# aayush9400/3D-Condtional-Stable-Diffusion

Measured on AMD Instinct MI355X. Metric: latent volumes/sec at 32^3x8ch T=1000 DDPM, higher is better.
Workload: dtype f32 (f16 hi+lo x3 MFMA, f32 accumulate)

## Files before the change

3d-condtional-stable-diffusion_amd/_lib.py:

```python
from __future__ import annotations

import ctypes as C
import os

_HERE = os.path.dirname(os.path.abspath(__file__))
LIB_PATH = os.environ.get("DM3D_LIB") or os.path.join(_HERE, "csrc", "libdm3d_hip.so")

ACT_NONE, ACT_RELU, ACT_SILU = 0, 1, 2
ABI_VERSION = 111
PREC_F32, PREC_H3 = 0, 1
WL_TAP, WL_PAIR = 0, 1
FMT_F32, FMT_H2 = 0, 1
COUT_PAD, CIN_PAD = 64, 16

_f32p = C.c_void_p
_i32p = C.c_void_p


class ConvDesc(C.Structure):
    _fields_ = [
        ("x1", _f32p), ("x2", _f32p), ("c1", C.c_int32), ("c2", C.c_int32), ("batch", C.c_int32),
        ("in_d", C.c_int32), ("in_h", C.c_int32), ("in_w", C.c_int32), ("upsample", C.c_int32),
        ("ksize", C.c_int32), ("stride", C.c_int32), ("wpk", _f32p), ("bias", _f32p),
        ("pro_scale", _f32p), ("pro_shift", _f32p), ("vec", _f32p), ("vec_idx", _i32p), ("vec_ld", C.c_int32),
# ... 152 lines not shown
    "dm3d_split_h2": (C.c_int, [_f32p, C.c_int64, C.c_int32, C.c_int64, C.c_int32, C.c_void_p, C.c_int64, C.c_void_p]),
    "dm3d_layernorm3_h2": (C.c_int, [_f32p, C.c_int64, C.c_int32, C.c_float] + [_f32p] * 9 + [C.c_void_p]),
    "dm3d_softmax_rows_h2": (C.c_int, [_f32p, C.c_int64, C.c_int32, C.c_int64, C.c_void_p]),
    "dm3d_layernorm3": (C.c_int, [_f32p, C.c_int64, C.c_int32, C.c_float] + [_f32p] * 9 + [C.c_void_p]),
    "dm3d_groupnorm_stats": (C.c_int, [_f32p, C.c_int32, C.c_int64, C.c_int32, C.c_void_p, C.c_int32, C.c_int32, C.c_void_p]),
    "dm3d_groupnorm_finalize": (C.c_int, [C.c_void_p, C.c_int32, C.c_int64, C.c_int32, C.c_int32, C.c_float, _f32p, _f32p, _f32p,
                                           _f32p, C.c_void_p]),
    "dm3d_groupnorm_finalize2": (C.c_int, [C.c_void_p, C.c_int32, C.c_void_p, C.c_int32, C.c_int32, C.c_int64, C.c_int32, C.c_float, _f32p, _f32p,
                                          _f32p, _f32p, C.c_void_p]),
    "dm3d_groupnorm_partials": (C.c_int, [_f32p, C.c_int32, C.c_int64, C.c_int32, C.c_void_p, C.c_void_p]),
    "dm3d_groupnorm_partials_bytes": (C.c_int64, [C.c_int32, C.c_int64, C.c_int32]),
    "dm3d_affine_act_batched": (C.c_int, [_f32p, _f32p, C.c_int32, C.c_int64, C.c_int32, _f32p, _f32p, C.c_int32, C.c_void_p]),
    "dm3d_softmax_rows": (C.c_int, [_f32p, C.c_int64, C.c_int32, C.c_int64, C.c_void_p]),
    "dm3d_affine_act": (C.c_int, [_f32p, _f32p, C.c_int64, C.c_int32, _f32p, _f32p, C.c_int32, C.c_void_p]),
    "dm3d_ddpm_update": (C.c_int, [C.POINTER(DdpmDesc), C.c_void_p]),
    "dm3d_ddim_update": (C.c_int, [C.POINTER(DdimDesc), C.c_void_p]),
    "dm3d_dpm_update": (C.c_int, [C.POINTER(DpmDesc), C.c_void_p]),
    "dm3d_edit_update": (C.c_int, [C.POINTER(EditDesc), C.c_void_p]),
    "dm3d_guide_update": (C.c_int, [C.POINTER(GuideDesc), C.c_void_p]),
    "dm3d_range_check": (C.c_int, [_f32p, C.c_int64, C.c_float, C.c_void_p, C.c_void_p]),
    "dm3d_add_i32": (C.c_int, [_i32p, C.c_int32, C.c_int32, C.c_void_p]),
    "dm3d_randn": (C.c_int, [_f32p, C.c_int64, C.c_uint64, C.c_uint32, C.c_void_p]),
    "dm3d_gather_rows": (C.c_int, [_f32p, C.c_int32, _i32p, _f32p, C.c_int32, C.c_int32, C.c_void_p]),
    "dm3d_vq_assign": (C.c_int, [_f32p, C.c_int64, C.c_int32, _f32p, C.c_int32, _f32p, _i32p, C.c_void_p]),
    "dm3d_batchnorm_finalize": (C.c_int, [C.c_void_p, C.c_int32, C.c_int64, C.c_int32, C.c_float] + [_f32p] * 8 + [C.c_float, C.c_int32, C.c_void_p]),
    "dm3d_affine_act_cat": (C.c_int, [_f32p, C.c_int32, _f32p, C.c_int32, C.c_int64, _f32p, _f32p, C.c_int32, _f32p, C.c_void_p]),
    "dm3d_bn_act_bwd": (C.c_int, [_f32p, _f32p, C.c_int32, _f32p, C.c_int32, C.c_int64, _f32p, _f32p, _f32p, _f32p, C.c_int32, C.c_void_p,
                                   _f32p, _f32p, _f32p, _f32p, C.c_void_p]),
    "dm3d_wgrad": (C.c_int, [C.POINTER(WgradDesc), C.c_void_p]),
    "dm3d_colsum": (C.c_int, [_f32p, C.c_int64, C.c_int64, C.c_int32, _f32p, C.c_int64, C.c_void_p]),
# ... 77 lines not shown
```

3d-condtional-stable-diffusion_amd/csrc/dm3d_conv.hip:

```cpp
#include <cstdlib>
#include "dm3d_conv_args.h"
#include <math.h>

namespace {

template <int TD, int TH, int TW, int S, int KS, int WM, int WN>
__global__ __launch_bounds__(256, 2) void conv3d_igemm_f32(const ConvArgs p) {
    constexpr int CK = 16, LDV = CK + 4, NT = 64;
    constexpr int TM = TD * TH * TW;
    constexpr int HD = (TD - 1) * S + KS, HH = (TH - 1) * S + KS, HW = (TW - 1) * S + KS;
    constexpr int HVOX = HD * HH * HW;
    constexpr int TAPS = KS * KS * KS;
    constexpr int MR = TM / WM / 32, NR = NT / WN / 32;
    constexpr int NTHR = WM * WN * 64;
    constexpr int NSLOT = (HVOX * 4 + NTHR - 1) / NTHR;
    static_assert(NTHR == 256, "kernel assumes 4 waves");
    static_assert(TM % (WM * 32) == 0 && NT % (WN * 32) == 0, "tile split");

    extern __shared__ __attribute__((aligned(16))) float smem[];
    float* lds_in = smem;
    float* lds_w = smem + HVOX * LDV;

    const int tid = threadIdx.x;
    const int lane = tid & 63, wave = tid >> 6;
// ... 169 lines not shown
    int dev_ = 0;
    DM3D_HIP(hipGetDevice(&dev_));
    DM3D_REQUIRE(dev_ >= 0 && dev_ < 64, "conv: device ordinal %d", dev_);
    if (!attr_set[dev_]) {
        DM3D_HIP(hipFuncSetAttribute(reinterpret_cast<const void*>(&conv3d_igemm_f32<TD, TH, TW, S, KS, WM, WN>),
                                     hipFuncAttributeMaxDynamicSharedMemorySize, (int)lds));
        attr_set[dev_] = true;
    }
    dim3 grid((unsigned)(a.batch * a.bd * a.bh * a.bw), (unsigned)(a.coutpad / 64), a.parity ? 8u : 1u);
    hipLaunchKernelGGL((conv3d_igemm_f32<TD, TH, TW, S, KS, WM, WN>), grid, dim3(256), lds, st, a);
    return dm3d_launch_check("conv3d_igemm_f32");
}

}

extern "C" int dm3d_conv3d_ndhwc(const dm3d_conv_desc* d, void* stream) {
    DM3D_REQUIRE(d != nullptr, "conv: null descriptor");
    DM3D_REQUIRE(d->x1 && d->wpk && d->out, "conv: x1/wpk/out must be non-null");
    DM3D_REQUIRE(d->ksize == 1 || d->ksize == 3 || (d->ksize == 4 && d->stride == 2), "conv: ksize %d not in {1,3} (4 needs stride 2)", d->ksize);
    DM3D_REQUIRE(d->stride == 1 || d->stride == 2, "conv: stride %d not in {1,2}", d->stride);
    DM3D_REQUIRE(!d->transpose || (d->ksize == 4 && d->stride == 2 && !d->upsample), "conv: transpose needs ksize 4, stride 2, no upsample");
    DM3D_REQUIRE(!(d->upsample && d->stride != 1), "conv: upsample requires stride 1");
    DM3D_REQUIRE(!(d->ksize == 1 && (d->stride != 1 || d->upsample)), "conv: ksize 1 supports stride 1 without upsample only");
    DM3D_REQUIRE(d->batch > 0 && d->in_d > 0 && d->in_h > 0 && d->in_w > 0 && d->cout > 0, "conv: non-positive extent");
    DM3D_REQUIRE(d->c1 > 0 && d->c1 % 4 == 0 && d->c2 >= 0 && d->c2 % 4 == 0, "conv: c1=%d c2=%d must be multiples of 4", d->c1, d->c2);
    DM3D_REQUIRE((d->c2 == 0) == (d->x2 == nullptr), "conv: x2 and c2 must be given together");
    DM3D_REQUIRE(d->c2 == 0 || d->c1 % 16 == 0, "conv: with a second input c1=%d must be a multiple of 16", d->c1);
    DM3D_REQUIRE((d->pro_scale == nullptr) == (d->pro_shift == nullptr), "conv: pro_scale and pro_shift go together");
    DM3D_REQUIRE(!d->vec || d->vec_ld >= d->cout, "conv: vec_ld %d < cout %d", d->vec_ld, d->cout);
    const void* ptrs[] = {d->x1, d->x2, d->wpk, d->pro_scale, d->pro_shift, d->out, d->res};
    for (const void* q : ptrs) DM3D_REQUIRE(dm3d_aligned16(q), "conv: pointer %p is not 16-byte aligned", q);
// ... 68 lines not shown
    a.out_scale = d->precision == DM3D_PREC_H3 ? ldexpf(1.0f, -d->w_exp) : 1.0f;
    hipStream_t st = static_cast<hipStream_t>(stream);
    const int which = par_mode ? DM3D_CONV_UP
                               : (d->ksize == 1 ? DM3D_CONV_K1 : (d->ksize == 4 ? DM3D_CONV_K4S2 : (d->stride == 2 ? DM3D_CONV_K3S2 : DM3D_CONV_K3S1)));
    if (par_mode) a.w_parity_stride = d->precision == DM3D_PREC_H3
        ? dm3d_packed_weight_h3_bytes(8, cin, d->cout) / 2 : dm3d_packed_weight_elems(8, cin, d->cout);
    if (d->gn_stats) {
        DM3D_REQUIRE(d->out_fmt == DM3D_FMT_F32 && d->cout % 4 == 0 && dm3d_aligned16(d->gn_stats),
                     "conv: gn_stats needs a float32 output, cout %% 4 == 0 and a 16-byte aligned buffer");
        a.gn_stats = d->gn_stats;
    }
    auto stats_behind = [&](int rc) {
        if (rc != DM3D_OK || !a.gn_stats) return rc;
        return dm3d_groupnorm_partials(a.out, a.batch, (int64_t)a.fd * a.fh * a.fw, a.cout, a.gn_stats, stream);
    };
    if (d->precision != DM3D_PREC_H3) return stats_behind(dm3d_conv_launch_f32(a, which, st));
    const int layout = dm3d_conv_weight_layout(d->ksize, d->stride, d->upsample, d->transpose, d->cout);
    DM3D_REQUIRE(d->w_layout == layout, "conv: w_layout %d but this geometry reads layout %d (dm3d_conv_weight_layout)", d->w_layout, layout);
    if (layout != DM3D_WL_PAIR) return stats_behind(dm3d_conv_launch_h3(a, which, st));
    if (dm3d_conv_h3w_serves(a, which)) return dm3d_conv_launch_h3w(a, which, st);
    return dm3d_conv_launch_h3v3(a, which, st);
}

extern "C" int64_t dm3d_packed_weight_skip_h3p_bytes(int32_t cin, int32_t cout) {
    return (cin > 0 && cout > 0) ? dm3d_h3v2_skip_image_bytes(cin, cout) : 0;
}

extern "C" int dm3d_pack_weights_skip_h3p(const float* keras_kernel, int32_t cin, int32_t cout, int32_t w_exp, void* packed, void* stream) {
    DM3D_REQUIRE(keras_kernel && packed && cin > 0 && cout > 0, "pack_weights_skip_h3p: bad arguments");
    DM3D_REQUIRE(w_exp >= -100 && w_exp <= 100 && dm3d_aligned16(packed), "pack_weights_skip_h3p: w_exp out of range or packed unaligned");
    return dm3d_pack_skip_h3v2(keras_kernel, cin, cout, w_exp, packed, static_cast<hipStream_t>(stream));
}

extern "C" int dm3d_pack_weights_skip_h3f(const float* keras_kernel, int32_t cin, int32_t cout, int32_t w_exp, void* packed, void* stream) {
    DM3D_REQUIRE(keras_kernel && packed && cin > 0 && cout > 0, "pack_weights_skip_h3f: bad arguments");
    DM3D_REQUIRE(w_exp >= -100 && w_exp <= 100 && dm3d_aligned16(packed), "pack_weights_skip_h3f: w_exp out of range or packed unaligned");
// ... 100 lines not shown
```

3d-condtional-stable-diffusion_amd/csrc/dm3d_conv_args.h:

```cpp
#pragma once
#include "dm3d_common.h"

struct ConvArgs {
    const float* x1; const float* x2; int c1, c2;
    int ind, inh, inw;
    int lgd, lgh, lgw;
    int od, oh, ow;
    int padz, pady, padx;
    int os;
    int ooz, ooy, oox;
    int fd, fh, fw;
    int parity;
    long w_parity_stride;
    const void* wpk; int cinpad, coutpad;
    const float* bias; const float* pscale; const float* pshift; long pro_bstride;
    const float* vec; const int* vec_idx; int vec_ld;
    int relu; const float* res; float* out; int cout;
    const float* prelu; int relu_out;
    int bd, bh, bw;
    int nchunks;
    int batch;
    float out_scale;
    int ksplit;
    int* split_counters;
    int split_counter_words;
    long split_tile_floats;
    void* scratch; long scratch_bytes;
    const float* post_scale; const float* post_shift;
    int out_h2;
    int x_h2;
    const float* sx1; const float* sx2; int sc1, sc2; const void* swpk; int s_npairs;
    const void* swpk_f;
    const void* wpk_wino;
    int* range_flag; float range_limit;
    float* gn_stats;
    int epi_vec4;
};

enum { DM3D_CONV_K3S1 = 0, DM3D_CONV_K3S2 = 1, DM3D_CONV_K1 = 2, DM3D_CONV_UP = 3, DM3D_CONV_K4S2 = 4 };

int dm3d_conv_launch_f32(ConvArgs& a, int which, hipStream_t st);
int dm3d_conv_launch_h3(ConvArgs& a, int which, hipStream_t st);
int dm3d_conv_launch_h3v3(ConvArgs& a, int which, hipStream_t st);
struct H3v2Launch { ConvArgs k; bool stats_after; };
int dm3d_h3v2_pre_launch(ConvArgs& a, int td, H3v2Launch& L, hipStream_t st, int force_ksplit = 0);
int dm3d_h3v2_post_launch(const ConvArgs& a, const H3v2Launch& L, hipStream_t st);
int dm3d_conv_h3v2_ksplit(const ConvArgs& a);
long dm3d_conv_split_tiles(const ConvArgs& a, int td);
int dm3d_conv_h3v3_td(const ConvArgs& a);
int64_t dm3d_h3v2_skip_image_bytes(int cin, int cout);
int dm3d_pack_skip_h3v2(const float* keras_kernel, int cin, int cout, int w_exp, void* packed, hipStream_t st);
// ... 8 lines not shown
```

3d-condtional-stable-diffusion_amd/csrc/dm3d_conv_h3v2_parts.h:

```cpp
#pragma once
#include "dm3d_conv_args.h"
#include "dm3d_h3.h"
#include <type_traits>

namespace h3v2 {

constexpr int REC = DM3D_REC;
typedef float f32x4v __attribute__((ext_vector_type(4)));

__host__ __device__ constexpr int pi_pos(int c) {
    return c < 4 ? (c < 2 ? c : c + 2) : (c >= 12 ? (c < 14 ? c - 4 : c - 2) : (((c - 4) >> 1) * 4 + 2 + ((c - 4) & 1)));
}
__device__ __forceinline__ int dx_of_row(int i) { return (0x1320 >> ((i >> 2) * 4)) & 3; }

#define DM3D_MFMA3_TILES(acc, nb, al, ah, bl, bh)                                                        \
    _Pragma("unroll") for (int pi_ = 0; pi_ < 4; ++pi_)                                                  \
        _Pragma("unroll") for (int k_ = 0; k_ < 2; ++k_) {                                               \
            f32x4v& c_ = acc[pi_][(nb) * 2 + k_];                                                        \
            c_ = __builtin_amdgcn_mfma_f32_16x16x32_f16(al[pi_], bh[k_], c_, 0, 0, 0);                   \
            c_ = __builtin_amdgcn_mfma_f32_16x16x32_f16(ah[pi_], bl[k_], c_, 0, 0, 0);                   \
            c_ = __builtin_amdgcn_mfma_f32_16x16x32_f16(ah[pi_], bh[k_], c_, 0, 0, 0);                   \
        }

struct Brick {
// ... 401 lines not shown
        for (int ni = 0; ni < NCT; ++ni) {
            *reinterpret_cast<f32x4*>(dst + ni * 32) = f32x4{gn[ni * 8], gn[ni * 8 + 1], gn[ni * 8 + 2], gn[ni * 8 + 3]};
            *reinterpret_cast<f32x4*>(dst + ni * 32 + 4) = f32x4{gn[ni * 8 + 4], gn[ni * 8 + 5], gn[ni * 8 + 6], gn[ni * 8 + 7]};
        }
        for (int k = 1; k < slices; ++k) {
            float* dz = dst + (size_t)k * bh * bw * p.cout * 2;
#pragma unroll
            for (int ni = 0; ni < NCT; ++ni) {
                *reinterpret_cast<f32x4*>(dz + ni * 32) = f32x4{0.f, 0.f, 0.f, 0.f};
                *reinterpret_cast<f32x4*>(dz + ni * 32 + 4) = f32x4{0.f, 0.f, 0.f, 0.f};
            }
        }
    }
}

struct EpiVecs { f32x4 add, ps, pt; };
__device__ __forceinline__ EpiVecs epilogue_cq_vecs(const ConvArgs& p, const Brick& br, const int vrow) {
    int tid = threadIdx.x;
    asm volatile("" : "+v"(tid));
    const int n = br.ntile * 64 + (tid & 15) * 4;
    const f32x4 zero = {0.f, 0.f, 0.f, 0.f}, one = {1.f, 1.f, 1.f, 1.f};
    EpiVecs ev;
    ev.add = zero; ev.ps = one; ev.pt = zero;
    if (br.ntile * 64 + 64 <= p.cout && p.epi_vec4) {
        if (p.bias) ev.add = *reinterpret_cast<const f32x4*>(p.bias + n);
        if (p.vec) {
            const f32x4 vv = *reinterpret_cast<const f32x4*>(p.vec + (size_t)vrow * p.vec_ld + n);
#pragma unroll
            for (int c = 0; c < 4; ++c) ev.add[c] += vv[c];
        }
// ... 122 lines not shown
```

3d-condtional-stable-diffusion_amd/csrc/dm3d_conv_h3v3.hip:

```cpp
#include <cstdlib>
#include "dm3d_conv_h3v2_parts.h"

using namespace h3v2;

#ifdef DM3D_CLOCK_STAMPS
__device__ unsigned long long* g_dbg_stamps_c = nullptr;
extern "C" int dm3d_debug_set_stamps_conv(void* p) { return (int)hipMemcpyToSymbol(HIP_SYMBOL(g_dbg_stamps_c), &p, sizeof(p)); }
#define STAMP(i) do { const unsigned wg_ = blockIdx.x + gridDim.x * blockIdx.y; \
    if (g_dbg_stamps_c && threadIdx.x == 0 && blockIdx.z == 0 && wg_ < 4096) { \
    g_dbg_stamps_c[wg_ * 32 + (i)] = __builtin_amdgcn_s_memtime(); \
    if ((i) == 0) g_dbg_stamps_c[wg_ * 32 + 24] = __builtin_amdgcn_s_memrealtime(); \
    if ((i) == 20) g_dbg_stamps_c[wg_ * 32 + 26] = __builtin_amdgcn_s_memrealtime(); \
    if ((i) == 29) g_dbg_stamps_c[wg_ * 32 + 25] = __builtin_amdgcn_s_memrealtime(); \
    if ((i) == 1) g_dbg_stamps_c[wg_ * 32 + 30] = __builtin_amdgcn_s_memrealtime(); \
    if ((i) == 28) g_dbg_stamps_c[wg_ * 32 + 31] = __builtin_amdgcn_s_memrealtime(); } } while (0)
#else
#define STAMP(i) do { } while (0)
#endif

namespace {

template <int KS, int MODE, int TD, int NCT = 4>
__global__ __launch_bounds__(TD * 64, 2) void conv3d_igemm_h3v3(const ConvArgs p) {
    constexpr int TH = 8, TW = 8, CK = 16, NT = 64, NTHR = TD * 64;
// ... 322 lines not shown
    const Brick br = {b, oz0, oy0, ox0, ooz, ooy, oox, ntile, khalf};
    if constexpr (KS == 3 && NCT == 4) {
        skip_phase<TD>(p, smem_v3, acc, br);
    }
    STAMP(19);
    if (p.ksplit > 1) {
        const long tile = ((long)blockIdx.z * gridDim.x + brick_all) * ntiles + ntile;
        const SplitTile stile = split_tile(p, tile, khalf);
        split_store(stile, acc, 0);
        STAMP(20);
        if (!split_is_last(p, tile, reinterpret_cast<unsigned*>(smem_v3))) return;
        STAMP(21);
        split_gather(stile, p, khalf, acc, 0);
        STAMP(22);
    }
    if (p.gn_stats) {
        float gn[NCT * 8];
#pragma unroll
        for (int i = 0; i < NCT * 8; ++i) gn[i] = 0.0f;
        epilogue<TD, NCT>(p, acc, br, -1, 4, -1, gn);
        gn_flush<TD, NCT>(p, gn, br, threadIdx.x >> 6, 1);
    } else {
        epilogue<TD, NCT>(p, acc, br);
    }
    STAMP(29);
}

template <int KS, int MODE, int TD, int NCT = 4>
int launch_v3(ConvArgs& a, hipStream_t st) {
    constexpr int HREC = (TD - 1 + KS) * (7 + KS) * 12;
// ... 9 lines not shown
        attr_set[dev] = true;
    }
    H3v2Launch L;
    if (int rc = dm3d_h3v2_pre_launch(a, TD, L, st)) return rc;
    dim3 grid((unsigned)(a.batch * a.bd * a.bh * a.bw), (unsigned)(a.coutpad / 64 * a.ksplit), a.parity ? 8u : 1u);
    hipLaunchKernelGGL((conv3d_igemm_h3v3<KS, MODE, TD, NCT>), grid, dim3(TD * 64), lds, st, L.k);
    if (int rc = dm3d_launch_check("conv3d_igemm_h3v3")) return rc;
    return dm3d_h3v2_post_launch(a, L, st);
}

template <int KS, int MODE>
int launch_td(ConvArgs& a, hipStream_t st) {
    if constexpr (KS == 3) {
        if (a.cout <= 32) {
            DM3D_REQUIRE(a.s_npairs == 0 && !a.out_h2, "conv: the fused skip conv / hand-off output need cout > 32");
            return a.cout <= 16 ? launch_v3<KS, MODE, 4, 1>(a, st) : launch_v3<KS, MODE, 4, 2>(a, st);
        }
    }
    return dm3d_conv_h3v3_td(a) == 8 ? launch_v3<KS, MODE, 8>(a, st) : launch_v3<KS, MODE, 4>(a, st);
}

}

int dm3d_conv_h3v3_td(const ConvArgs& a) {
    const char* e = getenv("DM3D_CONV_V3_TD");
    const int mode = e ? atoi(e) : 0;
    if (mode == 4) return 4;
    if (mode != 8 && (a.parity || a.s_npairs > 0)) return 4;
    if ((a.out_h2 || a.post_scale) && a.od % 8 != 0) return 4;
    const long wgs = (long)a.batch * ((a.od + 7) / 8) * ((a.oh + 7) / 8) * ((a.ow + 7) / 8) * (a.coutpad / 64) * (a.parity ? 8 : 1);
    const char* w = getenv("DM3D_CONV_WIDE_WGS");
    return wgs >= (w ? atol(w) : 512L) ? 8 : 4;
}

int dm3d_conv_launch_h3v3(ConvArgs& a, int which, hipStream_t st) {
    if (which == DM3D_CONV_UP) return a.pscale ? launch_td<2, 1>(a, st) : launch_td<2, 0>(a, st);
    if (a.x_h2) return launch_td<3, 2>(a, st);
    return a.pscale ? launch_td<3, 1>(a, st) : launch_td<3, 0>(a, st);
}
```

3d-condtional-stable-diffusion_amd/csrc/dm3d_elem.hip:

```cpp
#include "dm3d_h3.h"
#include "dm3d_philox.h"

namespace {

__device__ __forceinline__ float wave_sum(float v) {
#pragma unroll
    for (int o = 32; o > 0; o >>= 1) v += __shfl_xor(v, o, 64);
    return v;
}
__device__ __forceinline__ float wave_max(float v) {
#pragma unroll
    for (int o = 32; o > 0; o >>= 1) v = fmaxf(v, __shfl_xor(v, o, 64));
    return v;
}

__global__ __launch_bounds__(256) void layernorm3_kernel(const float* __restrict__ x, long rows, int c, float eps,
                                                         const float* g1, const float* b1, float* o1,
                                                         const float* g2, const float* b2, float* o2,
                                                         const float* g3, const float* b3, float* o3) {
    const int lane = threadIdx.x & 63;
    const long row = (long)blockIdx.x * 4 + (threadIdx.x >> 6);
    if (row >= rows) return;
    const int nv = c >> 2;
    const f32x4* xr = reinterpret_cast<const f32x4*>(x + row * c);
// ... 382 lines not shown
        reinterpret_cast<f32x4*>(x)[i] = philox_normal4((uint64_t)i, stream_id, 0x5eedu, seed);
}

struct DdpmArgs {
    float* x; const float* eps; const float* noise;
    int batch; long per4;
    const int* t;
    const float *beta, *sqa, *ab, *abp, *sqab, *sqabp, *sq1ab;
    uint64_t seed; int mode;
    float* mean_out; float* var_out;
    const uint64_t* seed_dev; int timesteps;
};

__global__ __launch_bounds__(256) void ddpm_kernel(const DdpmArgs p) {
    const int b = blockIdx.y;
    const int t = min(max(p.t[b], 0), p.timesteps - 1);
    const uint64_t seed = p.seed_dev ? *p.seed_dev : p.seed;
    const float be = p.beta[t], sqa = p.sqa[t], ab = p.ab[t], abp = p.abp[t];
    const float sqab = p.sqab[t], sqabp = p.sqabp[t], sq1ab = p.sq1ab[t];
    const float one_m_ab = __fsub_rn(1.0f, ab), one_m_abp = __fsub_rn(1.0f, abp);
    const float c1 = __fdiv_rn(__fmul_rn(be, sqabp), one_m_ab);
    const float c2 = __fdiv_rn(__fmul_rn(one_m_abp, sqa), one_m_ab);
    const float var = __fdiv_rn(__fmul_rn(one_m_abp, be), one_m_ab);
    const float sigma = expf(__fmul_rn(0.5f, logf(fmaxf(var, 1e-20f))));
    if (p.mode == 0 && p.var_out && blockIdx.x == 0 && threadIdx.x == 0) p.var_out[b] = var;
    const long base = (long)b * p.per4;
    for (long i = (long)blockIdx.x * 256 + threadIdx.x; i < p.per4; i += (long)gridDim.x * 256) {
        const f32x4 x = reinterpret_cast<const f32x4*>(p.x)[base + i];
        const f32x4 e = reinterpret_cast<const f32x4*>(p.eps)[base + i];
        f32x4 mean;
#pragma unroll
        for (int k = 0; k < 4; ++k) {
            const float x0 = __fdiv_rn(__fsub_rn(x[k], __fmul_rn(sq1ab, e[k])), sqab);
            mean[k] = __fadd_rn(__fmul_rn(c1, x0), __fmul_rn(c2, x[k]));
        }
        if (p.mode == 0) {
            reinterpret_cast<f32x4*>(p.mean_out)[base + i] = mean;
            continue;
        }
        f32x4 z = {0.f, 0.f, 0.f, 0.f};
        if (t > 0) z = p.noise ? reinterpret_cast<const f32x4*>(p.noise)[base + i]
                               : philox_normal4((uint64_t)(base + i), (uint32_t)t, 0xd1f0u, seed);
        f32x4 o;
#pragma unroll
        for (int k = 0; k < 4; ++k) {
            const float cl = mean[k] != mean[k] ? mean[k] : fminf(fmaxf(mean[k], -1.0f), 1.0f);
            o[k] = __fadd_rn(cl, __fmul_rn(sigma, z[k]));
        }
        reinterpret_cast<f32x4*>(p.x)[base + i] = o;
    }
}

typedef unsigned int u32x4r __attribute__((ext_vector_type(4)));
__global__ __launch_bounds__(256) void range_check_kernel(const float* __restrict__ x, long n4, float limit, int* __restrict__ flag) {
    unsigned int amax = 0u;
    for (long i = (long)blockIdx.x * 256 + threadIdx.x; i < n4; i += (long)gridDim.x * 256) {
        const u32x4r v = reinterpret_cast<const u32x4r*>(x)[i];
        amax = max(max(amax, max(v[0] & 0x7fffffffu, v[1] & 0x7fffffffu)), max(v[2] & 0x7fffffffu, v[3] & 0x7fffffffu));
    }
    if (amax > __float_as_uint(limit)) *flag = 1;
}

__global__ void add_i32_kernel(int* p, int n, int delta) {
    const int i = blockIdx.x * blockDim.x + threadIdx.x;
// ... 296 lines not shown
```

3d-condtional-stable-diffusion_amd/diffusion.py:

```python
from __future__ import annotations

import ctypes as C
import math
from typing import Optional

import numpy as np
import torch

from . import _lib
from ._lib import DdimDesc, DdpmDesc, DpmDesc, EditDesc, GuideDesc, check, lib
from .betas import BETAS_FIELDS, Betas
from .unet import UNet
from .weights import UNetConfig


def ddim_timesteps(T: int, num_steps=None, timesteps=None) -> np.ndarray:
    T = int(T)
    if num_steps is not None and timesteps is not None:
        raise ValueError("give num_steps or timesteps, not both")
    if timesteps is not None:
        ts = np.asarray(timesteps).reshape(-1)
        if ts.size == 0 or not np.all(ts == np.round(ts)) or ts.min() < 0 or ts.max() >= T or np.any(np.diff(ts) <= 0):
            raise ValueError(f"timesteps must be strictly increasing integers in [0, {T})")
        return ts.astype(np.int64)
# ... 686 lines not shown
        else:
            smp = DdimEditSampler(self, shape, ctx, seed, use_graph and not eager, sched, full, eta=eta, clip_x0=clip_x0)
        smp.reset(x0.to(dev), keep, None if known_noise is None else known_noise[n].contiguous())
        n_steps = n if steps is None else min(int(steps), n)
        for k in range(n_steps):
            i = n - 1 - k
            smp.step(noise=None if noise is None else noise[i].contiguous(),
                     known_noise=None if known_noise is None else known_noise[i].contiguous())
        out = smp.x.clone()
        self.network.check_range(smp.plan)
        return out

    MAX_GRAPHS = 8

    def _capture(self, smp: "Sampler"):
        key = (id(smp.plan), smp.KIND)
        if key in self._graphs:
            self._graphs[key] = self._graphs.pop(key)
            return self._graphs[key][0]
        torch.cuda.synchronize()
        cap = torch.cuda.Stream()
        g = C.c_void_p()
        check(lib().dm3d_graph_begin(cap.cuda_stream), "graph_begin")
        try:
            smp._enqueue(cap.cuda_stream, smp.desc)
        finally:
            rc = lib().dm3d_graph_end(cap.cuda_stream, C.byref(g))
        check(rc, "graph_end")
        self._graphs[key] = (g, smp.desc, cap, smp.plan)
        while len(self._graphs) > self.MAX_GRAPHS:
            old = next(iter(self._graphs))
# ... 41 lines not shown
        self.seed = (model.fresh_seed() if seed is None else int(seed)) & (2 ** 64 - 1)
        net, T = model.network, model.timesteps
        self.plan = net.plan(shape[0] * self.COPIES, T, ctx_ids is not None and len(ctx_ids) > 1, purpose="sampler")
        plan = self.plan
        if getattr(plan, "_time_filled", None) is not net.P:
            net.fill_time_table(np.arange(T), plan.vec)
            plan._time_filled = net.P
        if ctx_ids is not None:
            plan.set_context(ctx_ids)
        if getattr(plan, "seed_buf", None) is None:
            plan.seed_buf = torch.zeros(1, dtype=torch.int64, device=model.device)
        plan._owner_gen = getattr(plan, "_owner_gen", 0) + 1
        self._gen = plan._owner_gen
        self.desc = self._desc()
        self.desc.seed_dev = plan.seed_buf.data_ptr()
        self._t = -1

    KIND = "ddpm"
    COPIES = 1

    def _head(self, t):
        return t

    @property
    def x(self):
        return self._head(self.plan.x)

    def _guide(self, st):
        """Between the U-Net and the update: nothing (a guided chain: eps <- the guided eps)."""

# ... 2 lines not shown

    def _desc(self, noise=None):
        return self.model._ddpm_desc(self.x, self._head(self.plan.eps), self.plan.t_idx, 1, noise=noise, seed=self.seed)

    def _own(self):
        if self._gen != self.plan._owner_gen:
            raise RuntimeError("this Sampler was retired: a newer Sampler (generate() call) took over its plan")

    def reset(self, x_T=None):
        self._own()
        T = self.model.timesteps
        self._start(x_T)
        self.plan.t_idx.fill_(T - 1)
        if self.plan.range_flag is not None:
            self.plan.range_flag.zero_()
        self._t = T - 1

    def _start(self, x_T):
        plan = self.plan
        st = torch.cuda.current_stream().cuda_stream
        seed_i64 = self.seed - (1 << 64) if self.seed >= (1 << 63) else self.seed
        plan.seed_buf.fill_(seed_i64)
        if x_T is not None:
            self.x.copy_(torch.as_tensor(x_T, dtype=torch.float32).reshape(self.shape))
        else:
            check(lib().dm3d_randn(self.x.data_ptr(), self.x.numel(), self.seed, 0x7fffffff, st), "randn")

    def _enqueue(self, st, desc):
        self.plan.run(st)
        push, pop = _lib.roctx()
        push("ddpm")
        self._guide(st)
        check(lib().dm3d_ddpm_update(C.byref(desc), st), "ddpm_update")
        self._mirror(st)
        check(lib().dm3d_add_i32(self.plan.t_idx.data_ptr(), self.plan.B, -1, st), "add_i32")
        pop()

    def prepare(self):
        if self.use_graph:
            self.model._capture(self)
        return self

    def step(self, noise=None):
        self._own()
        if self._t < 0:
            raise RuntimeError("the chain is finished (or was never started): call reset() before step()")
        st = torch.cuda.current_stream().cuda_stream
        if noise is not None:
# ... 321 lines not shown
```

3d-condtional-stable-diffusion_amd/unet.py:

```python
from __future__ import annotations

import ctypes as C
import os
from typing import Dict, List, Optional, Sequence

import numpy as np
import torch

from . import _lib
from ._lib import ACT_NONE, ACT_RELU, ACT_SILU, AttnFrontDesc, ConvDesc, GemmDesc, MlpDesc, check, lib
from .betas import time_embedding_table
from .weights import UNetConfig, keras_init_weights, upsample_parity_kernels, walk

BN_EPS = 1e-3
LN_EPS = 1e-3


def _stream() -> int:
    return torch.cuda.current_stream().cuda_stream


def _ptr(t: Optional[torch.Tensor], offset_elems: int = 0) -> Optional[int]:
    if t is None:
        return None
# ... 403 lines not shown
class Plan:

    def __init__(self, net: UNet, batch: int, vec_rows: int, per_sample_context: bool):
        self.net, self.B, self.per_sample_context = net, batch, per_sample_context
        cfg, dev = net.cfg, net.device
        S, Cc = cfg.img_size, cfg.img_channels
        self.ops: List[tuple] = []
        self._keep: List[object] = []
        self.x = torch.empty(batch, S, S, S, Cc, dtype=torch.float32, device=dev)
        self.eps = torch.empty_like(self.x)
        self.t_idx = torch.zeros(batch, dtype=torch.int32, device=dev)
        self.vec = torch.empty(vec_rows, net.temb_ld, dtype=torch.float32, device=dev)
        self.ctx_bufs: Dict[str, tuple] = {}
        self._gn_stats = {}
        self.range_flag = torch.zeros(1, dtype=torch.int32, device=dev) if net.precision == "h3" else None
        self.uses_wino = False
        self.split_counters = torch.zeros(4096, dtype=torch.int32, device=dev)
        self.range_limit = net.range_limit
        self._build()
        if self.range_flag is not None and self.uses_wino:
            self.range_limit = net._h3_range_limit(winograd=True)
            for d in self._keep:
                for one in (d if isinstance(d, C.Array) else (d,)):
                    if isinstance(one, (ConvDesc, GemmDesc, MlpDesc, AttnFrontDesc)) and one.range_flag:
                        one.range_limit = self.range_limit
        need = max([lib().dm3d_conv_scratch_bytes(C.byref(d)) for d in self._keep if isinstance(d, ConvDesc)] + [0])
        if need:
            self.scratch = torch.empty(need // 4, dtype=torch.float32, device=dev)
            for d in self._keep:
                if isinstance(d, ConvDesc):
# ... 116 lines not shown
        self.ops.append((lib().dm3d_gemm_tn, (C.byref(d),), kind,
                         {"desc": f"{kind} m={d.m} n={d.n} k={d.k} batch={d.batch}", "flops": 2.0 * d.m * d.n * d.k * d.batch}))

    def _gemm_group(self, problems):
        arr = (GemmDesc * len(problems))(*[self._guard(_gemm_desc(**kw)) for kw in problems])
        self._keep.append(arr)
        fl = sum(2.0 * d.m * d.n * d.k * d.batch for d in arr)
        desc = "gemm_h3 group[" + " | ".join(f"m={d.m} n={d.n} k={d.k} b={d.batch}" for d in arr) + "]"
        self.ops.append((lib().dm3d_gemm_tn_group, (arr, len(problems)), "gemm_h3", {"desc": desc, "flops": fl}))

    def _build(self):
        net, cfg, B = self.net, self.net.cfg, self.B
        P = net.P
        S = cfg.img_size
        if self.range_flag is not None:
            self.ops.append((lib().dm3d_range_check, (self.x.data_ptr(), self.x.numel(), 65504.0,
                                                       self.range_flag.data_ptr()), "range", {}))
        h = self._buf(B, S, S, S, cfg.first_conv_channels)
        self._conv(P["conv_in"], self.x, h, S)
        skips = [(h, cfg.first_conv_channels)]
        cur, cur_c, edge = h, cfg.first_conv_channels, S
        last = net.blocks[-1] if net.blocks else None
        final_handoff = (last is not None and last.kind == "res" and net.h2_handoff and cfg.norm == "batch" and net.precision == "h3"
                         and S % 8 == 0 and last.cout % 64 == 0 and B * (S ** 3 // 256) * (last.cout // 64) > 256
                         and lib().dm3d_conv_weight_layout(3, 1, 0, 0, last.cout) == _lib.WL_PAIR
                         and lib().dm3d_conv_weight_layout(3, 1, 0, 0, cfg.img_channels) == _lib.WL_PAIR)
        for blk in net.blocks:
            if blk.kind == "push":
                skips.append((cur, cur_c))
            elif blk.kind == "res":
# ... 4 lines not shown
                        raise AssertionError("skip channel mismatch")
                cur = self._res_block(blk, cur, blk.cin, x2, c2, edge, final_post=P["out.norm"] if (final_handoff and blk is last) else None)
                cur_c = blk.cout
            elif blk.kind == "attn":
                cur = self._cross_block(blk, cur, edge) if cfg.conditional else self._self_block(blk, cur, edge)
            elif blk.kind == "down":
                out = self._buf(B, blk.edge, blk.edge, blk.edge, blk.cout)
                self._conv(P[blk.name], cur, out, edge, stride=2)
                cur, edge = out, blk.edge
            elif blk.kind == "up":
                out = self._buf(B, blk.edge, blk.edge, blk.edge, blk.cout)
                self._conv(P[blk.name], cur, out, edge, upsample=1)
                cur, edge = out, blk.edge
        if final_handoff:
            self._conv(P["out.conv"], cur, self.eps, edge, x1_h2=True, normed=False)
            return
        pro, bs = self._norm("out.norm", cur, cur_c, edge)
        self._conv(P["out.conv"], cur, self.eps, edge, pro=pro, pro_bstride=bs, normed=False)

    def _res_block(self, blk, x1, c1, x2, c2, edge, final_post=None):
        P, B, n, w = self.net.P, self.B, blk.name, blk.cout
        skip = None
        if f"{n}.skip_fused" in P:
            res, skip = None, (x1, x2, c1, c2, P[f"{n}.skip_fused"], P.get(f"{n}.skip_frag"))
        elif f"{n}.skip" in P:
            res = self._buf(B, edge, edge, edge, w)
            self._conv(P[f"{n}.skip"], x1, res, edge, x2=x2, c1=c1, c2=c2, normed=False)
        else:
            res = x1
        hmid = self._buf(B, edge, edge, edge, w)
        pro, bs = self._norm(f"{n}.norm1", x1, c1, edge, x2, c2)
        out = self._buf(B, edge, edge, edge, w)
        handoff = (self.net.h2_handoff and self.net.cfg.norm == "batch" and self.net.precision == "h3" and edge % 8 == 0
# ... 229 lines not shown

    def set_context(self, ctx_ids):
        ids = torch.as_tensor(np.asarray(ctx_ids, dtype=np.int32)).to(self.net.device)
        self._keep_ids = ids
        st = _stream()
        for n, (kbuf, vbuf) in self.ctx_bufs.items():
            ktab, vtab = self.net.ctx_tables[n]
            for tab, buf in ((ktab, kbuf), (vtab, vbuf)):
                check(lib().dm3d_gather_rows(tab.data_ptr(), tab.shape[0], ids.data_ptr(), buf.data_ptr(), buf.shape[0],
                                             buf.shape[1], st), "gather_rows")

    _RANGE_OF = {"conv_wino": "conv", "conv_wino_h2in": "conv", "conv_k3s1_td4": "conv", "conv_k1": "conv", "conv_k3s2": "conv", "conv_up": "conv", "conv_k3s1_n32": "conv", "conv_k3s1_h2in": "conv", "conv_k3s1": "conv",
                 "gemm": "attn", "gemm_h3": "attn", "mlp_fused": "attn", "attn_front": "attn", "attn_fused": "attn", "softmax": "attn", "layernorm": "attn", "groupnorm": "norm", "affine": "norm",
                 "range": "guard"}

    def run(self, stream: Optional[int] = None):
        st = _stream() if stream is None else stream
        push, pop = _lib.roctx()
        cur = None
        for fn, args, what, _ in self.ops:
            rng = self._RANGE_OF.get(what, what)
            if rng != cur:
                if cur is not None:
                    pop()
                push(rng)
                cur = rng
            rc = fn(*args, st)
            if rc != 0:
                pop()
                check(rc, what)
        if cur is not None:
            pop()

    def run_timed(self):
        st = _stream()
        evs = []
        for fn, args, what, meta in self.ops:
            e0, e1 = torch.cuda.Event(enable_timing=True), torch.cuda.Event(enable_timing=True)
            e0.record()
            rc = fn(*args, st)
            e1.record()
            if rc != 0:
                check(rc, what)
            evs.append((what, meta, e0, e1))
        torch.cuda.synchronize()
        return [(what, meta, e0.elapsed_time(e1)) for what, meta, e0, e1 in evs]

    def count(self) -> Dict[str, int]:
        out: Dict[str, int] = {}
        for _, _, what, _ in self.ops:
            out[what] = out.get(what, 0) + 1
        return out
# ... 1 lines not shown
```

include/dm3d.h:

```cpp
#ifndef DM3D_H
#define DM3D_H

#include <stdint.h>

#ifdef __cplusplus
extern "C" {
#endif

#define DM3D_VERSION 111

#define DM3D_OK            0
#define DM3D_EINVAL       -1
#define DM3D_EUNSUPPORTED -2
#define DM3D_EHIP         -3

#define DM3D_ACT_NONE 0
#define DM3D_ACT_RELU 1
#define DM3D_ACT_SILU 2

#define DM3D_PREC_F32 0
#define DM3D_PREC_H3  1

#define DM3D_FMT_F32 0
#define DM3D_FMT_H2  1
// ... 182 lines not shown
    const float* eps;
    const float* noise;
    int32_t batch; int64_t per_sample;
    const int32_t* t;
    int32_t timesteps;
    const float *beta, *sqrt_alpha, *alpha_bar, *alpha_bar_prev, *sqrt_alpha_bar, *sqrt_alpha_bar_prev,
                *sqrt_one_minus_alpha_bar;
    uint64_t seed;
    int32_t mode;
    float* mean_out; float* var_out;
    const uint64_t* seed_dev;
} dm3d_ddpm_desc;

int dm3d_ddpm_update(const dm3d_ddpm_desc* d, void* stream);

typedef struct dm3d_ddim_desc {
    float* x;
    const float* eps;
    const float* noise;
    float* out;
    int32_t batch; int64_t per_sample;
    const float* coef;
    const int32_t* tau;
    const int32_t* t_next;
    int32_t rows;
    const int32_t* pos;
    int32_t* t_idx;
    uint64_t seed;
    const uint64_t* seed_dev;
    int32_t mode;
// ... 112 lines not shown
```

Measured before the change: 2.309.

## Fuse DDPM update into output conv epilogue and drop per-step head range check

Adds a conv entry point whose H3 k3/stride-1 epilogue computes the predicted noise, applies the DDPM posterior mean, adds Philox noise and writes x in place. This removes the separate ddpm_update launch and the eps round trip through memory each timestep. It also folds the x range guard into the epilogue, skipping the head range_check op, with a single check run at reset. The fast path only applies in limited cases: mode 1 without injected noise, batch norm, cout <= 16, and whole 4x8x8 bricks. It also skips the guidance hook on the fused path.

```diff
diff --git a/3d-condtional-stable-diffusion_amd/_lib.py b/3d-condtional-stable-diffusion_amd/_lib.py
--- a/3d-condtional-stable-diffusion_amd/_lib.py
+++ b/3d-condtional-stable-diffusion_amd/_lib.py
@@ -190,6 +190,7 @@
     "dm3d_softmax_rows": (C.c_int, [_f32p, C.c_int64, C.c_int32, C.c_int64, C.c_void_p]),
     "dm3d_affine_act": (C.c_int, [_f32p, _f32p, C.c_int64, C.c_int32, _f32p, _f32p, C.c_int32, C.c_void_p]),
     "dm3d_ddpm_update": (C.c_int, [C.POINTER(DdpmDesc), C.c_void_p]),
+    "dm3d_conv3d_ddpm_tail": (C.c_int, [C.POINTER(ConvDesc), C.POINTER(DdpmDesc), C.c_float, C.c_void_p]),
     "dm3d_ddim_update": (C.c_int, [C.POINTER(DdimDesc), C.c_void_p]),
     "dm3d_dpm_update": (C.c_int, [C.POINTER(DpmDesc), C.c_void_p]),
     "dm3d_edit_update": (C.c_int, [C.POINTER(EditDesc), C.c_void_p]),
diff --git a/3d-condtional-stable-diffusion_amd/csrc/dm3d_conv.hip b/3d-condtional-stable-diffusion_amd/csrc/dm3d_conv.hip
--- a/3d-condtional-stable-diffusion_amd/csrc/dm3d_conv.hip
+++ b/3d-condtional-stable-diffusion_amd/csrc/dm3d_conv.hip
@@ -207,7 +207,7 @@
 
 }
 
-extern "C" int dm3d_conv3d_ndhwc(const dm3d_conv_desc* d, void* stream) {
+static int conv3d_impl(const dm3d_conv_desc* d, const DdpmTail* tail, void* stream) {
     DM3D_REQUIRE(d != nullptr, "conv: null descriptor");
     DM3D_REQUIRE(d->x1 && d->wpk && d->out, "conv: x1/wpk/out must be non-null");
     DM3D_REQUIRE(d->ksize == 1 || d->ksize == 3 || (d->ksize == 4 && d->stride == 2), "conv: ksize %d not in {1,3} (4 needs stride 2)", d->ksize);
@@ -306,12 +306,39 @@
         if (rc != DM3D_OK || !a.gn_stats) return rc;
         return dm3d_groupnorm_partials(a.out, a.batch, (int64_t)a.fd * a.fh * a.fw, a.cout, a.gn_stats, stream);
     };
+    if (tail) {
+        if (d->precision != DM3D_PREC_H3 || which != DM3D_CONV_K3S1 || d->out_fmt != DM3D_FMT_F32 ||
+            dm3d_conv_weight_layout(d->ksize, d->stride, d->upsample, d->transpose, d->cout) != DM3D_WL_PAIR)
+            return dm3d_fail(DM3D_EUNSUPPORTED, "conv: the DDPM tail needs a DM3D_PREC_H3 k3 / stride-1 conv in the DM3D_WL_PAIR layout with a float32 output");
+        a.tail = *tail;
+    }
     if (d->precision != DM3D_PREC_H3) return stats_behind(dm3d_conv_launch_f32(a, which, st));
     const int layout = dm3d_conv_weight_layout(d->ksize, d->stride, d->upsample, d->transpose, d->cout);
     DM3D_REQUIRE(d->w_layout == layout, "conv: w_layout %d but this geometry reads layout %d (dm3d_conv_weight_layout)", d->w_layout, layout);
     if (layout != DM3D_WL_PAIR) return stats_behind(dm3d_conv_launch_h3(a, which, st));
     if (dm3d_conv_h3w_serves(a, which)) return dm3d_conv_launch_h3w(a, which, st);
     return dm3d_conv_launch_h3v3(a, which, st);
+}
+
+extern "C" int dm3d_conv3d_ndhwc(const dm3d_conv_desc* d, void* stream) { return conv3d_impl(d, nullptr, stream); }
+
+extern "C" int dm3d_conv3d_ddpm_tail(const dm3d_conv_desc* d, const dm3d_ddpm_desc* u, float x_range_limit, void* stream) {
+    DM3D_REQUIRE(d != nullptr && u != nullptr, "conv_ddpm_tail: null descriptor");
+    DM3D_REQUIRE(u->x && u->t && dm3d_aligned16(u->x), "conv_ddpm_tail: x/t must be non-null, x 16-byte aligned");
+    DM3D_REQUIRE(u->mode == 1 && !u->noise && !u->mean_out && !u->var_out,
+                 "conv_ddpm_tail: mode 1 without injected noise only (mode 0, noise, mean_out / var_out: dm3d_conv3d_ndhwc + dm3d_ddpm_update)");
+    DM3D_REQUIRE(u->beta && u->sqrt_alpha && u->alpha_bar && u->alpha_bar_prev && u->sqrt_alpha_bar && u->sqrt_alpha_bar_prev &&
+                 u->sqrt_one_minus_alpha_bar, "conv_ddpm_tail: a Betas table is null");
+    DM3D_REQUIRE(u->timesteps > 0, "conv_ddpm_tail: timesteps=%d", u->timesteps);
+    DM3D_REQUIRE(u->batch == d->batch && u->per_sample == (int64_t)d->in_d * d->in_h * d->in_w * d->cout,
+                 "conv_ddpm_tail: x [%d, %lld] is not the shape of the conv's output", u->batch, (long long)u->per_sample);
+    DM3D_REQUIRE(static_cast<const void*>(u->x) != d->x1 && static_cast<const void*>(u->x) != d->x2, "conv_ddpm_tail: x must not be an input of the conv");
+    DdpmTail t{};
+    t.x = u->x; t.t = u->t;
+    t.tab = DdpmTables{u->beta, u->sqrt_alpha, u->alpha_bar, u->alpha_bar_prev, u->sqrt_alpha_bar, u->sqrt_alpha_bar_prev, u->sqrt_one_minus_alpha_bar};
+    t.seed = u->seed; t.seed_dev = u->seed_dev; t.timesteps = u->timesteps;
+    t.x_limit = x_range_limit > 0.0f ? x_range_limit : 65504.0f;
+    return conv3d_impl(d, &t, stream);
 }
 
 extern "C" int64_t dm3d_packed_weight_skip_h3p_bytes(int32_t cin, int32_t cout) {
diff --git a/3d-condtional-stable-diffusion_amd/csrc/dm3d_conv_args.h b/3d-condtional-stable-diffusion_amd/csrc/dm3d_conv_args.h
--- a/3d-condtional-stable-diffusion_amd/csrc/dm3d_conv_args.h
+++ b/3d-condtional-stable-diffusion_amd/csrc/dm3d_conv_args.h
@@ -1,5 +1,6 @@
 #pragma once
 #include "dm3d_common.h"
+#include "dm3d_ddpm_math.h"
 
 struct ConvArgs {
     const float* x1; const float* x2; int c1, c2;
@@ -35,6 +36,7 @@
     int* range_flag; float range_limit;
     float* gn_stats;
     int epi_vec4;
+    DdpmTail tail;
 };
 
 enum { DM3D_CONV_K3S1 = 0, DM3D_CONV_K3S2 = 1, DM3D_CONV_K1 = 2, DM3D_CONV_UP = 3, DM3D_CONV_K4S2 = 4 };
diff --git a/3d-condtional-stable-diffusion_amd/csrc/dm3d_conv_h3v2_parts.h b/3d-condtional-stable-diffusion_amd/csrc/dm3d_conv_h3v2_parts.h
--- a/3d-condtional-stable-diffusion_amd/csrc/dm3d_conv_h3v2_parts.h
+++ b/3d-condtional-stable-diffusion_amd/csrc/dm3d_conv_h3v2_parts.h
@@ -439,6 +439,65 @@
     }
 }
 
+template <int TD>
+__device__ __forceinline__ void epilogue_ddpm_tail(const ConvArgs& p, f32x4v (&acc)[4][1], const Brick& br) {
+    const int lane = threadIdx.x & 63, wave = threadIdx.x >> 6;
+    const int row = lane & 15, g4 = lane >> 4;
+    const int k = row & 3, c4 = row & ~3;
+    const bool live = c4 < p.cout;
+    const int cc = live ? c4 : 0;
+    const bool b0 = (row & 1) != 0, b1 = (row & 2) != 0;
+    auto xor1 = [](float v) { return __builtin_bit_cast(float, __builtin_amdgcn_update_dpp(0, __builtin_bit_cast(int, v), 0xB1, 0xf, 0xf, false)); };
+    auto xor2 = [](float v) { return __builtin_bit_cast(float, __builtin_amdgcn_update_dpp(0, __builtin_bit_cast(int, v), 0x4E, 0xf, 0xf, false)); };
+    const DdpmTail& T = p.tail;
+    const int t = ddpm_clamp_t(T.t[br.b], T.timesteps);
+    const uint64_t seed = T.seed_dev ? *T.seed_dev : T.seed;
+    const DdpmCoef kf = ddpm_coef(T.tab, t);
+    const f32x4 zero = {0.f, 0.f, 0.f, 0.f};
+    const f32x4 add = p.bias ? *reinterpret_cast<const f32x4*>(p.bias + cc) : zero;
+    const int dxl = dx_of_row(4 * g4);
+    const long zrow = ((long)br.b * p.od + br.oz0 + wave) * p.oh;
+    f32x4* x4 = reinterpret_cast<f32x4*>(T.x);
+    long idx4[4];
+    f32x4 xv[4];
+#pragma unroll
+    for (int pi = 0; pi < 4; ++pi) {
+        const int oy = br.oy0 + 4 * (pi >> 1) + k, ox = br.ox0 + 4 * (pi & 1) + dxl;
+        idx4[pi] = (((zrow + oy) * p.ow + ox) * p.cout + cc) >> 2;
+        xv[pi] = x4[idx4[pi]];
+    }
+    float amax = 0.0f;
+    unsigned int xmax = 0u;
+#pragma unroll
+    for (int pi = 0; pi < 4; ++pi) {
+        float a[4] = {acc[pi][0][0], acc[pi][0][1], acc[pi][0][2], acc[pi][0][3]};
+        {
+            float s0 = b0 ? a[0] : a[1], s1 = b0 ? a[2] : a[3];
+            float r0 = xor1(s0), r1 = xor1(s1);
+            if (b0) { a[0] = r0; a[2] = r1; } else { a[1] = r0; a[3] = r1; }
+            s0 = b1 ? a[0] : a[2]; s1 = b1 ? a[1] : a[3];
+            r0 = xor2(s0); r1 = xor2(s1);
+            if (b1) { a[0] = r0; a[1] = r1; } else { a[2] = r0; a[3] = r1; }
+        }
+        f32x4 e;
+#pragma unroll
+        for (int j = 0; j < 4; ++j) {
+            e[j] = fmaf(a[j], p.out_scale, add[j]);
+            if (live) DM3D_AMAX(amax, e[j]);
+        }
+        const f32x4 mean = ddpm_mean4(kf, xv[pi], e);
+        f32x4 z = zero;
+        if (t > 0) z = ddpm_noise4((uint64_t)idx4[pi], t, seed);
+        const f32x4 o = ddpm_step4(kf, mean, z);
+        if (live) {
+            x4[idx4[pi]] = o;
+#pragma unroll
+            for (int j = 0; j < 4; ++j) xmax = max(xmax, __float_as_uint(o[j]) & 0x7fffffffu);
+        }
+    }
+    if (p.range_flag && (amax > p.range_limit || xmax > __float_as_uint(T.x_limit))) *p.range_flag = 1;
+}
+
 struct EpiVecs { f32x4 add, ps, pt; };
 __device__ __forceinline__ EpiVecs epilogue_cq_vecs(const ConvArgs& p, const Brick& br, const int vrow) {
     int tid = threadIdx.x;
diff --git a/3d-condtional-stable-diffusion_amd/csrc/dm3d_conv_h3v3.hip b/3d-condtional-stable-diffusion_amd/csrc/dm3d_conv_h3v3.hip
--- a/3d-condtional-stable-diffusion_amd/csrc/dm3d_conv_h3v3.hip
+++ b/3d-condtional-stable-diffusion_amd/csrc/dm3d_conv_h3v3.hip
@@ -360,6 +360,13 @@
         split_gather(stile, p, khalf, acc, 0);
         STAMP(22);
     }
+    if constexpr (KS == 3 && NCT == 1) {
+        if (p.tail.x) {
+            epilogue_ddpm_tail<TD>(p, acc, br);
+            STAMP(29);
+            return;
+        }
+    }
     if (p.gn_stats) {
         float gn[NCT * 8];
 #pragma unroll
@@ -399,6 +406,13 @@
     if constexpr (KS == 3) {
         if (a.cout <= 32) {
             DM3D_REQUIRE(a.s_npairs == 0 && !a.out_h2, "conv: the fused skip conv / hand-off output need cout > 32");
+            if (a.tail.x) {
+                if (!(a.cout <= 16 && a.cout % 4 == 0 && a.od % 4 == 0 && a.oh % 8 == 0 && a.ow % 8 == 0 && a.os == 1 && !a.vec && !a.relu && !a.res
+                      && !a.prelu && !a.relu_out && !a.post_scale && !a.gn_stats && dm3d_aligned16(a.bias)))
+                    return dm3d_fail(DM3D_EUNSUPPORTED, "conv: the DDPM tail needs cout %% 4 == 0 and <= 16 (have %d), extents of whole 4x8x8 bricks (%d %d %d), and a bias-only "
+                                     "epilogue", a.cout, a.od, a.oh, a.ow);
+                return launch_v3<KS, MODE, 4, 1>(a, st);
+            }
             return a.cout <= 16 ? launch_v3<KS, MODE, 4, 1>(a, st) : launch_v3<KS, MODE, 4, 2>(a, st);
         }
     }
@@ -419,6 +433,8 @@
 }
 
 int dm3d_conv_launch_h3v3(ConvArgs& a, int which, hipStream_t st) {
+    if (a.tail.x && !(which == DM3D_CONV_K3S1 && a.cout <= 32))
+        return dm3d_fail(DM3D_EUNSUPPORTED, "conv: the DDPM tail needs a k3 / stride-1 conv with cout <= 16 (have cout %d)", a.cout);
     if (which == DM3D_CONV_UP) return a.pscale ? launch_td<2, 1>(a, st) : launch_td<2, 0>(a, st);
     if (a.x_h2) return launch_td<3, 2>(a, st);
     return a.pscale ? launch_td<3, 1>(a, st) : launch_td<3, 0>(a, st);
diff --git a/3d-condtional-stable-diffusion_amd/csrc/dm3d_ddpm_math.h b/3d-condtional-stable-diffusion_amd/csrc/dm3d_ddpm_math.h
--- /dev/null
+++ b/3d-condtional-stable-diffusion_amd/csrc/dm3d_ddpm_math.h
@@ -0,0 +1,52 @@
+#pragma once
+#include "dm3d_philox.h"
+
+struct DdpmTables {
+    const float *beta, *sqa, *ab, *abp, *sqab, *sqabp, *sq1ab;
+};
+struct DdpmTail {
+    float* x; const int* t; DdpmTables tab;
+    uint64_t seed; const uint64_t* seed_dev; int timesteps;
+    float x_limit;
+};
+
+struct DdpmCoef { float c1, c2, var, sigma, sqab, sq1ab; };
+
+static __device__ __forceinline__ int ddpm_clamp_t(int t, int timesteps) { return min(max(t, 0), timesteps - 1); }
+
+static __device__ __forceinline__ DdpmCoef ddpm_coef(const DdpmTables& T, const int t) {
+    const float be = T.beta[t], sqa = T.sqa[t], ab = T.ab[t], abp = T.abp[t];
+    const float sqab = T.sqab[t], sqabp = T.sqabp[t], sq1ab = T.sq1ab[t];
+    const float one_m_ab = __fsub_rn(1.0f, ab), one_m_abp = __fsub_rn(1.0f, abp);
+    DdpmCoef k;
+    k.c1 = __fdiv_rn(__fmul_rn(be, sqabp), one_m_ab);
+    k.c2 = __fdiv_rn(__fmul_rn(one_m_abp, sqa), one_m_ab);
+    k.var = __fdiv_rn(__fmul_rn(one_m_abp, be), one_m_ab);
+    k.sigma = expf(__fmul_rn(0.5f, logf(fmaxf(k.var, 1e-20f))));
+    k.sqab = sqab; k.sq1ab = sq1ab;
+    return k;
+}
+
+static __device__ __forceinline__ f32x4 ddpm_mean4(const DdpmCoef& k, const f32x4 x, const f32x4 e) {
+    f32x4 mean;
+#pragma unroll
+    for (int i = 0; i < 4; ++i) {
+        const float x0 = __fdiv_rn(__fsub_rn(x[i], __fmul_rn(k.sq1ab, e[i])), k.sqab);
+        mean[i] = __fadd_rn(__fmul_rn(k.c1, x0), __fmul_rn(k.c2, x[i]));
+    }
+    return mean;
+}
+
+static __device__ __forceinline__ f32x4 ddpm_noise4(const uint64_t idx4, const int t, const uint64_t seed) {
+    return philox_normal4(idx4, (uint32_t)t, 0xd1f0u, seed);
+}
+
+static __device__ __forceinline__ f32x4 ddpm_step4(const DdpmCoef& k, const f32x4 mean, const f32x4 z) {
+    f32x4 o;
+#pragma unroll
+    for (int i = 0; i < 4; ++i) {
+        const float cl = mean[i] != mean[i] ? mean[i] : fminf(fmaxf(mean[i], -1.0f), 1.0f);
+        o[i] = __fadd_rn(cl, __fmul_rn(k.sigma, z[i]));
+    }
+    return o;
+}
diff --git a/3d-condtional-stable-diffusion_amd/csrc/dm3d_elem.hip b/3d-condtional-stable-diffusion_amd/csrc/dm3d_elem.hip
--- a/3d-condtional-stable-diffusion_amd/csrc/dm3d_elem.hip
+++ b/3d-condtional-stable-diffusion_amd/csrc/dm3d_elem.hip
@@ -1,5 +1,6 @@
 #include "dm3d_h3.h"
 #include "dm3d_philox.h"
+#include "dm3d_ddpm_math.h"
 
 namespace {
 
@@ -420,40 +421,23 @@
 
 __global__ __launch_bounds__(256) void ddpm_kernel(const DdpmArgs p) {
     const int b = blockIdx.y;
-    const int t = min(max(p.t[b], 0), p.timesteps - 1);
+    const int t = ddpm_clamp_t(p.t[b], p.timesteps);
     const uint64_t seed = p.seed_dev ? *p.seed_dev : p.seed;
-    const float be = p.beta[t], sqa = p.sqa[t], ab = p.ab[t], abp = p.abp[t];
-    const float sqab = p.sqab[t], sqabp = p.sqabp[t], sq1ab = p.sq1ab[t];
-    const float one_m_ab = __fsub_rn(1.0f, ab), one_m_abp = __fsub_rn(1.0f, abp);
-    const float c1 = __fdiv_rn(__fmul_rn(be, sqabp), one_m_ab);
-    const float c2 = __fdiv_rn(__fmul_rn(one_m_abp, sqa), one_m_ab);
-    const float var = __fdiv_rn(__fmul_rn(one_m_abp, be), one_m_ab);
-    const float sigma = expf(__fmul_rn(0.5f, logf(fmaxf(var, 1e-20f))));
-    if (p.mode == 0 && p.var_out && blockIdx.x == 0 && threadIdx.x == 0) p.var_out[b] = var;
+    const DdpmTables tab = {p.beta, p.sqa, p.ab, p.abp, p.sqab, p.sqabp, p.sq1ab};
+    const DdpmCoef kf = ddpm_coef(tab, t);
+    if (p.mode == 0 && p.var_out && blockIdx.x == 0 && threadIdx.x == 0) p.var_out[b] = kf.var;
     const long base = (long)b * p.per4;
     for (long i = (long)blockIdx.x * 256 + threadIdx.x; i < p.per4; i += (long)gridDim.x * 256) {
         const f32x4 x = reinterpret_cast<const f32x4*>(p.x)[base + i];
         const f32x4 e = reinterpret_cast<const f32x4*>(p.eps)[base + i];
-        f32x4 mean;
-#pragma unroll
-        for (int k = 0; k < 4; ++k) {
-            const float x0 = __fdiv_rn(__fsub_rn(x[k], __fmul_rn(sq1ab, e[k])), sqab);
-            mean[k] = __fadd_rn(__fmul_rn(c1, x0), __fmul_rn(c2, x[k]));
-        }
+        const f32x4 mean = ddpm_mean4(kf, x, e);
         if (p.mode == 0) {
             reinterpret_cast<f32x4*>(p.mean_out)[base + i] = mean;
             continue;
         }
         f32x4 z = {0.f, 0.f, 0.f, 0.f};
-        if (t > 0) z = p.noise ? reinterpret_cast<const f32x4*>(p.noise)[base + i]
-                               : philox_normal4((uint64_t)(base + i), (uint32_t)t, 0xd1f0u, seed);
-        f32x4 o;
-#pragma unroll
-        for (int k = 0; k < 4; ++k) {
-            const float cl = mean[k] != mean[k] ? mean[k] : fminf(fmaxf(mean[k], -1.0f), 1.0f);
-            o[k] = __fadd_rn(cl, __fmul_rn(sigma, z[k]));
-        }
-        reinterpret_cast<f32x4*>(p.x)[base + i] = o;
+        if (t > 0) z = p.noise ? reinterpret_cast<const f32x4*>(p.noise)[base + i] : ddpm_noise4((uint64_t)(base + i), t, seed);
+        reinterpret_cast<f32x4*>(p.x)[base + i] = ddpm_step4(kf, mean, z);
     }
 }
 
diff --git a/3d-condtional-stable-diffusion_amd/diffusion.py b/3d-condtional-stable-diffusion_amd/diffusion.py
--- a/3d-condtional-stable-diffusion_amd/diffusion.py
+++ b/3d-condtional-stable-diffusion_amd/diffusion.py
@@ -2,6 +2,7 @@
 
 import ctypes as C
 import math
+import os
 from typing import Optional
 
 import numpy as np
@@ -724,7 +725,7 @@
     MAX_GRAPHS = 8
 
     def _capture(self, smp: "Sampler"):
-        key = (id(smp.plan), smp.KIND)
+        key = (id(smp.plan), smp.KIND, bool(getattr(smp, "_fused", False)))
         if key in self._graphs:
             self._graphs[key] = self._graphs.pop(key)
             return self._graphs[key][0]
@@ -796,6 +797,7 @@
         self._gen = plan._owner_gen
         self.desc = self._desc()
         self.desc.seed_dev = plan.seed_buf.data_ptr()
+        self._fused = self.KIND == "ddpm" and plan.tail_ok and os.environ.get("DM3D_FUSED_TAIL", "1") != "0"
         self._t = -1
 
     KIND = "ddpm"
@@ -828,6 +830,9 @@
         self.plan.t_idx.fill_(T - 1)
         if self.plan.range_flag is not None:
             self.plan.range_flag.zero_()
+        if self._fused:
+            check(lib().dm3d_range_check(self.x.data_ptr(), self.x.numel(), 65504.0, self.plan.range_flag.data_ptr(),
+                                         torch.cuda.current_stream().cuda_stream), "range_check")
         self._t = T - 1
 
     def _start(self, x_T):
@@ -841,11 +846,13 @@
             check(lib().dm3d_randn(self.x.data_ptr(), self.x.numel(), self.seed, 0x7fffffff, st), "randn")
 
     def _enqueue(self, st, desc):
-        self.plan.run(st)
+        fused = self._fused and not desc.noise
+        self.plan.run(st, tail=desc if fused else None)
         push, pop = _lib.roctx()
         push("ddpm")
-        self._guide(st)
-        check(lib().dm3d_ddpm_update(C.byref(desc), st), "ddpm_update")
+        if not fused:
+            self._guide(st)
+            check(lib().dm3d_ddpm_update(C.byref(desc), st), "ddpm_update")
         self._mirror(st)
         check(lib().dm3d_add_i32(self.plan.t_idx.data_ptr(), self.plan.B, -1, st), "add_i32")
         pop()
diff --git a/3d-condtional-stable-diffusion_amd/unet.py b/3d-condtional-stable-diffusion_amd/unet.py
--- a/3d-condtional-stable-diffusion_amd/unet.py
+++ b/3d-condtional-stable-diffusion_amd/unet.py
@@ -441,6 +441,8 @@
         self.ctx_bufs: Dict[str, tuple] = {}
         self._gn_stats = {}
         self.range_flag = torch.zeros(1, dtype=torch.int32, device=dev) if net.precision == "h3" else None
+        self._head_guard = self._out_conv = None
+        self.tail = None
         self.uses_wino = False
         self.split_counters = torch.zeros(4096, dtype=torch.int32, device=dev)
         self.range_limit = net.range_limit
@@ -587,6 +589,7 @@
         P = net.P
         S = cfg.img_size
         if self.range_flag is not None:
+            self._head_guard = len(self.ops)
             self.ops.append((lib().dm3d_range_check, (self.x.data_ptr(), self.x.numel(), 65504.0,
                                                        self.range_flag.data_ptr()), "range", {}))
         h = self._buf(B, S, S, S, cfg.first_conv_channels)
@@ -621,9 +624,13 @@
                 cur, edge = out, blk.edge
         if final_handoff:
             self._conv(P["out.conv"], cur, self.eps, edge, x1_h2=True, normed=False)
-            return
-        pro, bs = self._norm("out.norm", cur, cur_c, edge)
-        self._conv(P["out.conv"], cur, self.eps, edge, pro=pro, pro_bstride=bs, normed=False)
+        else:
+            pro, bs = self._norm("out.norm", cur, cur_c, edge)
+            self._conv(P["out.conv"], cur, self.eps, edge, pro=pro, pro_bstride=bs, normed=False)
+        Cc = cfg.img_channels
+        if (net.precision == "h3" and cfg.norm == "batch" and self.range_flag is not None and edge == S and S % 8 == 0 and Cc % 4 == 0
+                and Cc <= 16 and lib().dm3d_conv_weight_layout(3, 1, 0, 0, Cc) == _lib.WL_PAIR):
+            self._out_conv = len(self.ops) - 1
 
     def _res_block(self, blk, x1, c1, x2, c2, edge, final_post=None):
         P, B, n, w = self.net.P, self.B, blk.name, blk.cout
@@ -883,11 +890,27 @@
                  "gemm": "attn", "gemm_h3": "attn", "mlp_fused": "attn", "attn_front": "attn", "attn_fused": "attn", "softmax": "attn", "layernorm": "attn", "groupnorm": "norm", "affine": "norm",
                  "range": "guard"}
 
-    def run(self, stream: Optional[int] = None):
+    @property
+    def tail_ok(self) -> bool:
+        return self._out_conv is not None
+
+    def _launches(self, guard: bool = True):
+        for i, op in enumerate(self.ops):
+            if self.tail is not None:
+                if i == self._head_guard and not guard:
+                    continue
+                if i == self._out_conv:
+                    op = (lib().dm3d_conv3d_ddpm_tail, (op[1][0], C.byref(self.tail), 65504.0)) + op[2:]
+            yield op
+
+    def run(self, stream: Optional[int] = None, tail=None):
+        if tail is not None and not self.tail_ok:
+            raise _lib.Dm3dError("this plan's output conv cannot carry the DDPM update")
+        self.tail = tail
         st = _stream() if stream is None else stream
         push, pop = _lib.roctx()
         cur = None
-        for fn, args, what, _ in self.ops:
+        for fn, args, what, _ in self._launches(guard=False):
             rng = self._RANGE_OF.get(what, what)
             if rng != cur:
                 if cur is not None:
@@ -904,7 +927,7 @@
     def run_timed(self):
         st = _stream()
         evs = []
-        for fn, args, what, meta in self.ops:
+        for fn, args, what, meta in self._launches():
             e0, e1 = torch.cuda.Event(enable_timing=True), torch.cuda.Event(enable_timing=True)
             e0.record()
             rc = fn(*args, st)
diff --git a/include/dm3d.h b/include/dm3d.h
--- a/include/dm3d.h
+++ b/include/dm3d.h
@@ -220,6 +220,8 @@
 
 int dm3d_ddpm_update(const dm3d_ddpm_desc* d, void* stream);
 
+int dm3d_conv3d_ddpm_tail(const dm3d_conv_desc* d, const dm3d_ddpm_desc* u, float x_range_limit, void* stream);
+
 typedef struct dm3d_ddim_desc {
     float* x;
     const float* eps;
```

Measured after the change: 2.309, median of 2. No clear change (-0.0%).
